# tphakala/birdnet-go

Measured on AMD Instinct MI355X. Metric: 3s-48kHz clips/sec (whole node) + max-abs prob diff vs TFLite, BirdNET v2.4, higher is better.
Workload: dtype f32; 1 GPU; BASELINE configs[1]: BirdNET v2.4 fp32, batch 256 x 3 s @ 48 kHz per GPU, mel front-end + CNN + head on device, raw logits out; batch_per_gpu=256, n_samples=144000, n_classes=6522, pipeline_depth=2, input_sets=4

## Files before the change

birdnet-go_amd/csrc/engine.cpp:

```cpp
#include "engine.h"

#include <algorithm>
#include <cmath>
#include <cstdio>
#include <cstdlib>
#include <cstring>
#include <mutex>
#include <sstream>

#include "../../include/bnhip.h"
#include "hostpipe.h"

namespace bnhip {

#define HIPCHK(call)                                                                           \
    do {                                                                                       \
        hipError_t e_ = (call);                                                                \
        if (e_ != hipSuccess) {                                                                \
            *err = std::string(#call) + ": " + hipGetErrorString(e_);                          \
            return false;                                                                      \
        }                                                                                      \
    } while (0)

Engine::~Engine() {
// ... 383 lines not shown
        if (s.kind == S_MEAN_FINISH && si > 1 && steps[si - 2].tail == 1 && tail_taken(si - 2, n, nl > 1)) continue;
        ProfEntry pe{};
        static const char* dbg_sync_before = getenv("BNHIP_DEBUG_SYNC_BEFORE");
        static const char* dbg_sync_after = getenv("BNHIP_DEBUG_SYNC_AFTER");
        static const char* dbg_ctx1_only = getenv("BNHIP_DEBUG_CTX1_ONLY");
        if (dbg_ctx1_only && cur_ctx == 1 && !strstr(dbg_ctx1_only, s.kclass)) continue;
        static const char* dbg_ctx1_skip = getenv("BNHIP_DEBUG_CTX1_SKIP");
        if (dbg_ctx1_skip && cur_ctx == 1 && strstr(dbg_ctx1_skip, s.kclass)) continue;
        if (dbg_sync_before && (!strcmp(dbg_sync_before, s.kclass) || s.name.rfind(dbg_sync_before, 0) == 0)) hipStreamSynchronize(stream);
        const bool prof_this = profiling && (profile_filter.empty() || profile_filter == s.kclass);
        if (prof_this) { pe.a = get_event(); pe.b = get_event(); pe.step = si; pe.n = n; hipEventRecord(pe.a, stream); }
        switch (s.kind) {
            case S_MINMAX:
                launch_clip_minmax(in0, n, n_samples, specs[0].eps, reinterpret_cast<float2*>(out),
                                   mm_scratch ? mm_scratch + ((size_t)std::max(cur_ctx, 0) * kMaxLanes + (size_t)li) * kMinMaxScratch : nullptr, stream);
                break;
            case S_FRONTEND: {
                const FrontSpec& fs = specs[s.spec];
                FrontendParams p;
                p.x = in0; p.mm = reinterpret_cast<const float2*>(in1); p.G = fs.G; p.window = fs.window; p.out = out;
                p.n_samples = n_samples; p.L = fs.L; p.Lfft = fs.Lfft; p.Kp = fs.Kp; p.hop = fs.hop; p.F = fs.F; p.n_mels = fs.n_mels;
                p.NTP = fs.NTP; p.C = C_spec; p.c = fs.c; p.norm_sub = fs.norm_sub; p.norm_mul = fs.norm_mul;
                p.p1 = fs.p1; p.p2 = fs.p2; p.n_clips = n;
                launch_frontend(p, stream);
                break;
            }
            case S_NORMALIZE:
                launch_normalize(in0, reinterpret_cast<const float2*>(in1), out, n, n_samples, specs[0].norm_sub, specs[0].norm_mul, stream);
                break;
            case S_STFT: {
                const FrontSpec& fs = specs[s.spec];
                StftParams p{in0, fs.window_full, fs.bins, out, n_samples, fs.Lfft, fs.L, fs.hop, fs.F, fs.nb, fs.nbp, fs.mode, n, fs.stft_tw, fs.pad_left};
                p.zmask = fs.stft_zmask;
                if (s.mode == 1) {
                    p.out = nullptr; p.img = out; p.mel = s.w3; p.mel_quads = s.S; p.n_mels = fs.n_mels; p.Ctot = C_spec; p.c0 = fs.c;
                    p.logc = fs.log_compress ? 1 : 0; p.time_major = fs.time_major ? 1 : 0; p.p1 = fs.p1; p.p2 = fs.p2;
                    p.lfloor = fs.log_floor; p.lscale = fs.log_scale;
                }
                {
                    static const bool f32_off = getenv("BNHIP_STFT_F32") && atoi(getenv("BNHIP_STFT_F32")) == 0;
                    if (precision == 1 && s.mode != 1 && fs.log_compress && !f32_off) p.f32 = 1;
                }
                launch_stft_bins(p, stream);
                break;
            }
            case S_MELBAND: {
                const FrontSpec& fa = specs[s.spec];
                const FrontSpec& fb = specs[s.S == 2 ? s.op : s.spec];
                MelBandParams p{{in0, s.S == 2 ? in1 : in0}, {s.w0, s.S == 2 ? s.w2 : s.w0},
                                {reinterpret_cast<const int*>(s.w1), reinterpret_cast<const int*>(s.S == 2 ? s.w3 : s.w1)},
                                {fa.nbp, fb.nbp}, {fa.p1, fb.p1}, {fa.p2, fb.p2}, out, fa.F, fa.n_mels, C_spec, fa.c,
                                fa.log_compress ? 1 : 0, fa.log_floor, fa.log_scale, fa.time_major ? 1 : 0};
                launch_mel_banded(p, s.S, n, stream);
                break;
            }
            case S_MELFIN: {
                const FrontSpec& fa = specs[s.spec];
                const FrontSpec& fb = specs[s.S == 2 ? s.op : s.spec];
                MelFinParams p{{in0, s.S == 2 ? in1 : in0}, {fa.p1, fb.p1}, {fa.p2, fb.p2}, out, fa.F, fa.n_mels, fa.n_mels, C_spec, fa.c,
                               fa.log_compress ? 1 : 0, fa.log_floor, fa.log_scale, fa.time_major ? 1 : 0};
                launch_mel_finish(p, s.S, n, stream);
                break;
            }
            case S_CONV_DIRECT: {
                ConvParams p{in0, s.w0, s.w1, out, n, s.H, s.W, s.C, s.Ho, s.Wo, s.Co, s.kh, s.kw, s.sh, s.sw, s.pt, s.pl, s.act};
                p.out_bf16 = vals[s.out].half ? 1 : 0;
// ... 137 lines not shown

static void jesc(std::ostringstream& os, const std::string& s) {
    for (char c : s) { if (c == '"' || c == '\\') os << '\\'; os << c; }
}

struct StepView { std::string name; double flops, bytes; bool absorbed; };
static StepView step_view(const Engine& e, size_t i) {
    const Step& s = e.steps[i];
    StepView v{s.name, s.flops, s.bytes, false};
    auto fused = [&](size_t k) { return e.steps[k].kind == S_PW && e.steps[k].tail && e.steps[k].wm_full >= 13; };
    if (fused(i)) {
        const double mine = 4.0 * s.H * s.W * s.Co;
        if (s.tail == 2) { v.name += "+dw"; v.flops += e.steps[i + 1].flops; }
        else { v.name += "+mean"; v.flops += e.steps[i + 1].flops + e.steps[i + 2].flops; v.bytes += 4.0 * s.Co - mine; }
    } else if ((s.kind == S_DW && i > 0 && e.steps[i - 1].tail == 2 && fused(i - 1)) ||
               (s.kind == S_MEAN_PARTIAL && i > 0 && e.steps[i - 1].tail == 1 && fused(i - 1)) ||
               (s.kind == S_MEAN_FINISH && i > 1 && e.steps[i - 2].tail == 1 && fused(i - 2))) {
        v.flops = 0; v.bytes = 0; v.absorbed = true;
    }
    return v;
}

std::string Engine::describe() const {
    std::ostringstream os;
    os << "{\"tune_source\":\"";
    jesc(os, tune_source);
    os << "\",\"tune_key\":\"" << (device >= 0 ? tune_key() : std::string()) << "\",\"split_step\":" << split_step << ",\"heatmap_tail\":\"" << (heatmap_pruned_step() >= 0 ? "pruned" : "gather") << "\",\"n_samples\":" << n_samples << ",\"n_classes\":" << n_classes << ",\"emb_dim\":" << emb_dim
       << ",\"max_batch\":" << max_batch << ",\"logits_output\":" << logits_output << ",\"embedding_output\":" << embedding_output << ",\"precision\":\"" << (precision ? "bf16" : "f32") << "\",\"lanes\":" << n_lanes << ",\"lane_min_batch\":" << dual_lane_min << ",\"act_arena_bytes\":" << act_bytes << ",\"weight_bytes\":" << w_bytes
       << ",\"specs\":[";
    for (size_t i = 0; i < specs.size(); i++) {
        const FrontSpec& f = specs[i];
        os << (i ? "," : "") << "{\"frame_length\":" << f.L << ",\"fft_length\":" << f.Lfft << ",\"hop\":" << f.hop
           << ",\"frames\":" << f.F << ",\"n_mels\":" << f.n_mels << ",\"channel\":" << f.c << ",\"p1\":" << f.p1
           << ",\"p2\":" << f.p2 << "}";
    }
    os << "],\"steps\":[";
    for (size_t i = 0; i < steps.size(); i++) {
        const Step& s = steps[i];
        const StepView sv = step_view(*this, i);
        const bool absorbed = sv.absorbed;
        os << (i ? "," : "") << "{\"i\":" << i << ",\"kernel\":\"" << s.kclass << "\",\"name\":\"";
        jesc(os, sv.name);
        os << "\",\"H\":" << s.H << ",\"W\":" << s.W << ",\"C\":" << s.C << ",\"Co\":" << s.Co << ",\"k\":" << s.kh
           << ",\"stride\":" << s.sh << ",\"act\":" << s.act << ",\"fused_scale\":" << (s.kind == S_PW && s.in1 >= 0 ? 1 : 0)
           << ",\"shape\":" << s.shape << ",\"dw_lds\":" << s.dwl << ",\"bx\":" << s.bx << ",\"nt\":" << s.nt << ",\"wm\":" << s.wm << ",\"nt_full\":" << s.nt_full << ",\"wm_full\":" << s.wm_full << ",\"fused_res\":" << (s.kind == S_PW && s.in2 >= 0 ? 1 : 0) << ",\"fused_sum\":" << (s.out2 >= 0 ? 1 : 0) << ",\"flops\":" << sv.flops << ",\"bytes\":" << sv.bytes << ",\"wbytes\":" << s.wbytes
           << ",\"tail\":" << s.tail << ",\"absorbed\":" << (absorbed ? 1 : 0) << ",\"out_v\":" << s.out << ",\"out2_v\":" << s.out2
           << ",\"in_bf16\":" << ((s.in0 >= 0 && vals[s.in0].half) ? 1 : 0) << ",\"out_bf16\":" << ((s.out >= 0 && vals[s.out].half) ? 1 : 0) << "}";
    }
    os << "]}";
    return os.str();
}

std::string Engine::profile_read() {
    hipStreamSynchronize(stream);
    struct Agg { double ms = 0, flops = 0, bytes = 0; long launches = 0; };
    std::map<std::string, Agg> agg;
    std::vector<std::string> order;
    std::vector<Agg> per_step(steps.size());
    for (auto& e : prof) {
        float ms = 0;
        hipEventElapsedTime(&ms, e.a, e.b);
        const Step& s = steps[e.step];
        const StepView sv = step_view(*this, e.step);
        if (!agg.count(s.kclass)) order.push_back(s.kclass);
        Agg& a = agg[s.kclass];
        a.ms += ms; a.launches++; a.flops += sv.flops * e.n; a.bytes += sv.bytes * e.n + s.wbytes;
        Agg& ps = per_step[e.step];
        ps.ms += ms; ps.launches++; ps.flops += sv.flops * e.n; ps.bytes += sv.bytes * e.n + s.wbytes;
        ev_pool.push_back(e.a); ev_pool.push_back(e.b);
    }
    prof.clear();
    std::ostringstream os;
    os << "[";
    for (size_t i = 0; i < order.size(); i++) {
        const Agg& a = agg[order[i]];
        os << (i ? "," : "") << "{\"kernel\":\"" << order[i] << "\",\"launches\":" << a.launches << ",\"ms\":" << a.ms
           << ",\"flops\":" << a.flops << ",\"bytes\":" << a.bytes << "}";
    }
    for (size_t i = 0; i < steps.size(); i++) {
        const Agg& a = per_step[i];
// ... 11 lines not shown
```

birdnet-go_amd/csrc/engine.h:

```cpp
#pragma once
#include <hip/hip_runtime.h>

#include <map>
#include <string>
#include <vector>

#include "kernels.h"
#include "tflite_model.h"

namespace bnhip {

enum StepKind { S_MINMAX, S_FRONTEND, S_NORMALIZE, S_STFT, S_MELFIN, S_MELBAND, S_CONV_DIRECT, S_PW, S_DW, S_EXPAND_DW, S_MEAN_PARTIAL, S_MEAN_FINISH, S_SE, S_UNARY, S_BINARY,
                S_EW_UNARY, S_EW_BINARY, S_POOL, S_COPY, S_SOFTMAX, S_REDUCE, S_CONV_GENERIC,
                S_CONV_IGEMM };

struct GenGeom {
    int d[4] = {1, 1, 1, 1};
    long sa[4] = {0, 0, 0, 0}, sb[4] = {0, 0, 0, 0}, so[4] = {0, 0, 0, 0};
    long offa = 0, offo = 0;
    bool a_const = false, b_const = false;
    int mask = 0;
    float alpha = 0.f;
    bool fill = false;
    int dh = 1, dw = 1, depthwise = 0, mult = 1;
// ... 10 lines not shown
    int bx = 0;
    int H = 0, W = 0, C = 0, Ho = 0, Wo = 0, Co = 0, kh = 1, kw = 1, sh = 1, sw = 1, pt = 0, pl = 0;
    int act = 0, act2 = 0, op = 0, mode = 0, S = 1, Cr = 0;
    int nt = 0, wm = 0;
    int tail = 0;
    int H2 = 0, W2 = 0, pt2 = 0, pl2 = 0;
    int shape = -1;
    int nt_full = 0, wm_full = 0;
    int spec = -1;
    GenGeom g;
    double flops = 0, bytes = 0, wbytes = 0;
};

struct Value {
    int tfl = -1;
    size_t elems = 0;
    size_t offset = 0;
    size_t offset_lane = 0;
    int first = -1, last = -1;
    bool external = false;
    bool half = false;
};

struct FrontSpec {
    int L, Kp, Lfft, hop, F, n_mels, NTP, c;
    float p1, p2, eps, norm_sub, norm_mul;
    const double* G = nullptr;
    const float* window = nullptr;
    bool fft = false;
    int nb = 0, nbp = 0, mode = 0;
    const float* window_full = nullptr;
    const double* stft_tw = nullptr;
    unsigned stft_zmask = 0xffffffffu;
    const int* bins = nullptr;
    bool normalize = true, log_compress = false, time_major = false;
    int pad_left = 0;
    float log_floor = 0.f, log_scale = 1.f;
};

struct ProfEntry { hipEvent_t a, b; int step; int n; };

struct WeightPlan {
    std::vector<float> img;
    std::vector<size_t> step_w[4];
    std::vector<size_t> step_bx;
};

inline DwParams dw_params(const Step& s, const float* in = nullptr, float* out = nullptr, int n = 1) {
    return DwParams{in, s.w0, s.w1, out, n, s.H, s.W, s.C, s.Ho, s.Wo, s.kh, s.kw, s.sh, s.sw, s.pt, s.pl, s.act};
}
PwTail tail_of(const Step& s, const Step& c);

class Engine {
  public:
    ~Engine();
    bool build(TflModel m, int device, int max_batch, bool plan_only, std::string* err, int* code);
    bool run(const float* d_in, int n, float* d_logits, float* d_emb, std::string* err);

    int device = 0, max_batch = 256;
    bool no_reuse = false;
    bool autotune = true;
    bool defer_weights = false;
    void finish_deferred();
    char* weights_ptr() const { return w_arena; }
    size_t weights_bytes() const { return w_bytes; }
    int frontend_fft = -1;
// ... 114 lines not shown
```

birdnet-go_amd/csrc/kernels.h:

```cpp
#pragma once
#include <atomic>
#include <hip/hip_runtime.h>

#include <vector>
#include <cstdint>

namespace bnhip {

inline int device_cus() {
    static std::atomic<int> cus[64];
    int dev = 0;
    if (hipGetDevice(&dev) != hipSuccess) { (void)hipGetLastError(); return 256; }
    if (dev < 0 || dev >= 64) return 256;
    int c = cus[dev].load(std::memory_order_relaxed);
    if (c > 0) return c;
    hipDeviceProp_t pr{};
    if (hipGetDeviceProperties(&pr, dev) != hipSuccess || pr.multiProcessorCount <= 0) { (void)hipGetLastError(); return 256; }
    cus[dev].store(pr.multiProcessorCount, std::memory_order_relaxed);
    return pr.multiProcessorCount;
}

template <auto Kern>
inline void lds_limit_once(int bytes) {
    static std::atomic<unsigned long long> done{0};
// ... 9 lines not shown

enum Act : int { ACT_NONE = 0, ACT_RELU = 1, ACT_RELU_N1_TO_1 = 2, ACT_RELU6 = 3, ACT_TANH = 4, ACT_SWISH = 100, ACT_SIGMOID = 101, ACT_HARD_SWISH = 102 };

void launch_pcm_to_f32(const void* pcm, int bits , float* out, size_t n, hipStream_t s);

constexpr int kMinMaxParts = 16;
void launch_clip_minmax(const float* x, int n_clips, int n_samples, float eps, float2* mm, float* scratch , hipStream_t s);

struct FrontendParams {
    const float* x;
    const float2* mm;
    const double* G;
    const float* window;
    float* out;
    int n_samples, L, Lfft, Kp, hop, F, n_mels, NTP, C, c;
    float norm_sub, norm_mul;
    float p1, p2;
    int n_clips;
};
void launch_frontend(const FrontendParams& p, hipStream_t s);
size_t frontend_lds_bytes(int Lfft, int Kp, int hop, int NTP);

struct StftParams {
    const float* xn;
    const float* window;
    const int* bins;
    float* out;
    int n_samples, Lfft, L, hop, F, nb, nbp, mode , n_clips;
    const double* tw = nullptr;
    int pad_left = 0;
    int nb_cap = 0, fpw = 0;
    int f32 = 0;
    unsigned zmask = 0xffffffffu;
    const float* mel = nullptr;
    int mel_quads = 0, n_mels = 0, Ctot = 1, c0 = 0, logc = 0, time_major = 0;
    float p1 = 1.f, p2 = 1.f, lfloor = 0.f, lscale = 1.f;
    float* img = nullptr;
};
std::vector<double> stft_build_tables(int Lfft, const int* bins, int nb);
unsigned stft_zmask(int Lfft, const int* bins, int nb);
std::vector<float> stft_mel_table(int Lfft, const float* melw, const int* span, int n_mels, int nb, int nbp, int* quads);
void launch_normalize(const float* x, const float2* mm, float* out, int n_clips, int n_samples, float norm_sub,
                      float norm_mul, hipStream_t s);
bool stft_supported(int Lfft, int nb);
void launch_stft_bins(const StftParams& p, hipStream_t s);
struct MelFinParams {
    const float* T[2];
    float p1[2], p2[2];
    float* out;
    int F, n_mels, ldt, Ctot, c0;
    int log = 0;
    float lfloor = 0.f, lscale = 1.f;
    int time_major = 0;
};
void launch_mel_finish(const MelFinParams& p, int nch, int n_clips, hipStream_t s);
struct MelBandParams {
    const float* bins[2];
    const float* w[2];
    const int* span[2];
    int nbp[2];
    float p1[2], p2[2];
    float* out;
    int F, n_mels, Ctot, c0;
    int log = 0;
    float lfloor = 0.f, lscale = 1.f;
    int time_major = 0;
};
bool mel_banded_supported(int n_mels, int nbp0, int nbp1);
void launch_mel_banded(const MelBandParams& p, int nch, int n_clips, hipStream_t s);
int frontend_kc(int Lfft, int hop, int NTP);

struct ConvParams {
    const float* in; const float* w ; const float* bias; float* out;
// ... 152 lines not shown
```

birdnet-go_amd/csrc/planner.cpp:

```cpp
#include "engine.h"

#include <algorithm>
#include <cmath>
#include <cstdio>
#include <cstdlib>
#include <cstring>
#include <map>

#include "../../include/bnhip.h"

namespace bnhip {

namespace {

size_t align_up(size_t v, size_t a) { return (v + a - 1) / a * a; }

struct Planner {
    const TflModel& m;
    std::vector<int> producer;
    std::vector<std::vector<int>> consumers;
    std::vector<int> uses;
    std::vector<char> absorbed;
    std::string err;

// ... 260 lines not shown
        return P.fail("front-end: unexpected spectrogram tensor shape");
    fm->out_tensor = t;
    return true;
}

std::vector<double> build_G(const Planner& P, const FrontendMatch& fm, const std::vector<int>& krows, int Kp, int NTP) {
    const int nb = fm.Lfft / 2 + 1, nm = fm.n_mels, N = fm.Lfft;
    const float* melT = P.T(fm.mel_tensor).f32();
    std::vector<double> ctab(N);
    for (int i = 0; i < N; i++) ctab[i] = std::cos(2.0 * M_PI * (double)i / (double)N);
    std::vector<double> melk(krows.size() * (size_t)nm);
    for (size_t r = 0; r < krows.size(); r++)
        for (int mm = 0; mm < nm; mm++) melk[r * nm + mm] = (double)melT[(size_t)mm * nb + krows[r]];
    std::vector<double> G((size_t)Kp * NTP, 0.0);
    std::vector<double> row(nm);
    for (int n = 0; n <= fm.Lfft / 2; n++) {
        std::fill(row.begin(), row.end(), 0.0);
        for (size_t r = 0; r < krows.size(); r++) {
            double c = ctab[(size_t)(((long long)krows[r] * n) % N)];
            const double* mk = &melk[r * nm];
            for (int mm = 0; mm < nm; mm++) row[mm] += c * mk[mm];
        }
        for (int mo = 0; mo < nm; mo++) {
            int mm = fm.reverse ? nm - 1 - mo : mo;
            G[(size_t)n * NTP + mo] = row[mm];
        }
    }
    return G;
}

struct PlanSwitches {
    bool mel_banded = !getenv("BNHIP_NO_MEL_BANDED");
    bool fuse_mel = getenv("BNHIP_FUSE_MEL") != nullptr;
    bool fuse_expdw = !(getenv("BNHIP_NO_FUSE_EXPDW") && atoi(getenv("BNHIP_NO_FUSE_EXPDW")) != 0);
    bool conv_igemm = !getenv("BNHIP_NO_CONV_IGEMM");
    bool stem_mfma = !getenv("BNHIP_NO_STEM_MFMA");
    bool fuse_stem = !getenv("BNHIP_NO_FUSE_STEM");
};

int map_act(int fused, int* post = nullptr) {
    if (post) *post = 0;
    switch (fused) {
        case 0: return ACT_NONE; case 1: return ACT_RELU; case 3: return ACT_RELU6;
        case 2: if (post) { *post = U_RELU_N1_TO_1; return ACT_NONE; } return -1;
        case 4: if (post) { *post = U_TANH; return ACT_NONE; } return -1;
        default: return -1;
    }
}

void conv_pads(const TflOp& o, int H, int W, int Ho, int Wo, int kh, int kw, int* pt, int* pl) {
    *pt = 0; *pl = 0;
    if (o.explicit_pad) { *pt = o.pad_t; *pl = o.pad_l; return; }
    if (o.padding == 0) {
        *pt = std::max((Ho - 1) * o.stride_h + (kh - 1) * o.dil_h + 1 - H, 0) / 2;
        *pl = std::max((Wo - 1) * o.stride_w + (kw - 1) * o.dil_w + 1 - W, 0) / 2;
    }
}

bool shape5(const std::vector<int>& sh, int out[5]) {
    std::vector<int> v = sh;
    while (v.size() > 5 && v[0] == 1) v.erase(v.begin());
    if (v.size() > 5) return false;
    for (int k = 0; k < 5; k++) out[k] = 1;
    for (size_t k = 0; k < v.size(); k++) out[5 - v.size() + k] = v[k];
    return out[0] == 1;
}
// ... 237 lines not shown
            add_step(nz);
        }
        fs.nb = (int)bins.size(); fs.nbp = (int)align_up(fs.nb, 4); fs.mode = fm.magnitude ? 1 : 0;
        const int nbins = fm.Lfft / 2 + 1;
        const float* melT = P.T(fm.mel_tensor).f32();
        std::vector<float> melw((size_t)fm.n_mels * fs.nbp, 0.f);
        for (int mo = 0; mo < fm.n_mels; mo++) {
            int mm = fm.reverse ? fm.n_mels - 1 - mo : mo;
            for (int r = 0; r < fs.nb; r++) melw[(size_t)mo * fs.nbp + r] = melT[(size_t)mm * nbins + bins[r]];
        }
        const size_t o_win = wpush(fm.window), o_bins = wpush_i32(bins);
        const size_t o_mel = wpush(melw);
        std::vector<double> twt = stft_build_tables(fm.Lfft, bins.data(), fs.nb);
        fs.stft_zmask = stft_zmask(fm.Lfft, bins.data(), fs.nb);
        const size_t o_tw = wpush(reinterpret_cast<const float*>(twt.data()), twt.size() * 2);
        specs.push_back(fs);
        const int si = (int)specs.size() - 1;
        std::vector<int> span((size_t)2 * fm.n_mels, 0);
        long span_sum = 0;
        for (int mo = 0; mo < fm.n_mels; mo++) {
            int lo = fs.nb, hi = 0;
            for (int r = 0; r < fs.nb; r++)
                if (melw[(size_t)mo * fs.nbp + r] != 0.0f) { lo = std::min(lo, r); hi = r + 1; }
            if (hi == 0) lo = 0;
            span[2 * mo] = lo; span[2 * mo + 1] = hi;
            span_sum += hi - lo;
        }
        const size_t o_span = wpush_i32(span);
        const bool banded = sw.mel_banded && span_sum * 4 <= (long)fm.n_mels * fs.nb;
        int mel_quads = 0;
        std::vector<float> meltab;
        if (banded && sw.fuse_mel) meltab = stft_mel_table(fm.Lfft, melw.data(), span.data(), fm.n_mels, fs.nb, fs.nbp, &mel_quads);
        const bool fused = !meltab.empty();
        int v_bins = fused ? -1 : new_val(-1, (size_t)fm.F * fs.nbp);
        Step st; st.kind = S_STFT; st.name = "stft" + std::to_string(i); st.kclass = "stft"; st.in0 = v_xn; st.out = fused ? v_spec : v_bins;
        st.spec = si;
        st.flops = (double)fm.F * 2.5 * fm.Lfft * std::log2((double)fm.Lfft / 2);
        st.bytes = (double)E.n_samples * 4 + (double)fm.F * (fused ? fm.n_mels : fs.nbp) * 4;
        if (fused) { st.mode = 1; st.S = mel_quads; st.name += "+mel"; st.flops += 4.0 * fm.F * fs.nb; }
        add_step(st, o_win, o_bins, o_tw, fused ? wpush(meltab) : SIZE_MAX);
        fft_fin.push_back({v_bins, si, o_mel, o_span, banded, fused});
        return true;
    }
    bool gemm_channel(int i, FrontSpec fs, const std::vector<int>& bins) {
        const FrontendMatch& fm = fms[i];
        std::vector<double> G = build_G(P, fm, bins, fs.Kp, fs.NTP);
        const size_t goff = wpush(reinterpret_cast<const float*>(G.data()), G.size() * 2);
        std::vector<float> wpad((size_t)2 * fs.Kp, 0.0f);
        for (int n = 0; n <= fm.Lfft / 2; n++) {
            if (n < fm.L) wpad[n] = fm.window[n];
            int mi = fm.Lfft - n;
            if (n > 0 && mi != n && mi < fm.L) wpad[fs.Kp + n] = fm.window[mi];
        }
        const size_t woff = wpush(wpad);
        specs.push_back(fs);
        Step f; f.kind = S_FRONTEND; f.name = "melspec" + std::to_string(i); f.kclass = "frontend";
        f.in0 = E.v_input; f.in1 = E.v_mm; f.out = v_spec; f.spec = (int)specs.size() - 1;
        f.flops = 2.0 * fm.F * (fm.Lfft / 2 + 1) * fm.n_mels;
        f.bytes = (double)E.n_samples * 4 + (double)fm.F * fm.n_mels * 4;
        return add_step(f, goff, woff);
    }
    void mel_finish() {
        for (size_t k = 0; k < fft_fin.size();) {
            if (fft_fin[k].fused) { k++; continue; }
            const FrontSpec& a = specs[fft_fin[k].spec];
            const FrontSpec* b = k + 1 < fft_fin.size() && !fft_fin[k + 1].fused ? &specs[fft_fin[k + 1].spec] : nullptr;
// ... 856 lines not shown
```

birdnet-go_amd/csrc/stft.hip:

```cpp
#include "kernels.h"

#include <hip/hip_runtime.h>

#include <algorithm>
#include <vector>
#include <cmath>
#include <cstdio>
#include <cstdlib>

namespace bnhip {

__global__ void k_normalize(const float* __restrict__ x, const float2* __restrict__ mm, float* __restrict__ out,
                            int n_samples, float norm_sub, float norm_mul) {
    const int b = blockIdx.y;
    const float2 m = mm[b];
    const float* xc = x + (size_t)b * n_samples;
    float* oc = out + (size_t)b * n_samples;
    for (int i = blockIdx.x * blockDim.x + threadIdx.x; i < n_samples; i += gridDim.x * blockDim.x) {
        float t = xc[i] - m.x;
        t = t / m.y;
        t = t - norm_sub;
        oc[i] = t * norm_mul;
    }
}
// ... 12 lines not shown
    constexpr int LOG = P == 16 ? 4 : (P == 8 ? 3 : (P == 4 ? 2 : 1));
#pragma unroll
    for (int i = 0; i < P; i++) {
        int j = 0;
#pragma unroll
        for (int bit = 0; bit < LOG; bit++) j |= ((i >> bit) & 1) << (LOG - 1 - bit);
        if (i < j) { R t = re[i]; re[i] = re[j]; re[j] = t; t = im[i]; im[i] = im[j]; im[j] = t; }
    }
#pragma unroll
    for (int len = 2; len <= P; len <<= 1) {
        const int half = len >> 1, step = 16 / len;
#pragma unroll
        for (int i = 0; i < P; i += len) {
#pragma unroll
            for (int k = 0; k < half; k++) {
                const R wr = (R)C16[k * step], wi = (R)-S16[k * step];
                const R xr = re[i + k + half], xi = im[i + k + half];
                const R ur = re[i + k], ui = im[i + k];
                if (k == 0) {
                    re[i + k] = ur + xr; im[i + k] = ui + xi; re[i + k + half] = ur - xr; im[i + k + half] = ui - xi;
                } else if (2 * k == half) {
                    re[i + k] = ur + xi; im[i + k] = ui - xr; re[i + k + half] = ur - xi; im[i + k + half] = ui + xr;
                } else {
                    re[i + k] = fma(xr, wr, fma(-xi, wi, ur));
                    im[i + k] = fma(xr, wi, fma(xi, wr, ui));
                    re[i + k + half] = fma(-xr, wr, fma(xi, wi, ur));
                    im[i + k + half] = fma(-xr, wi, fma(-xi, wr, ui));
                }
            }
        }
    }
}

__device__ __forceinline__ float mel_pow(float v, float p1, float p2);
__device__ __forceinline__ float mel_log(float v, float lfloor, float lscale);

template <int P, int W, bool MEL = false, typename R = double>
__global__ __launch_bounds__(64 * W) void k_stft_bins(StftParams p) {
    constexpr int N2 = 64 * P;
    constexpr int N = 2 * N2;
    constexpr int Q = 64 / P;
    constexpr int RS = P == 8 ? 66 : 65;
    constexpr int WSZ = P * RS;
    constexpr int NPAIR = (P * P + 63) / 64;
    extern __shared__ __attribute__((aligned(16))) unsigned char stft_sm[];
    R* sm = reinterpret_cast<R*>(stft_sm);
    R* twr = sm;
    R* twi = twr + P * 64;
    R* t2r = twi + P * 64;
    R* t2i = t2r + Q * P;
    R* work = t2i + Q * P;
    float4* melw4 = reinterpret_cast<float4*>(work + (size_t)W * 2 * WSZ);
    const int* binq = reinterpret_cast<const int*>(melw4 + p.mel_quads);
    const int tid = threadIdx.x, lane = tid & 63, wave = tid >> 6;
    const int b = blockIdx.y;

    constexpr int NTAB = 2 * P * 64 + 2 * Q * P;
    for (int i = tid; i < NTAB; i += blockDim.x) sm[i] = (R)p.tw[i];
    int mA = 0, loA = 0, nA = 0, wA = 0, mB = 0, loB = 0, nB = 0, wB = 0;
    if (MEL) {
        const float4* src = reinterpret_cast<const float4*>(p.mel + 64 * 8);
        for (int i = tid; i < p.mel_quads + (p.mel_quads + 3) / 4; i += blockDim.x) melw4[i] = src[i];
        const int4* lt = reinterpret_cast<const int4*>(p.mel) + 2 * lane;
        const int4 ta = lt[0], tb = lt[1];
        mA = ta.x; loA = ta.y; nA = ta.z; wA = ta.w; mB = tb.x; loB = tb.y; nB = tb.z; wB = tb.w;
    }
    __syncthreads();

    R* wre = work + (size_t)wave * 2 * WSZ;
    R* wim = wre + WSZ;
    const float* xc = p.xn + (size_t)b * p.n_samples;
    float w0[P], w1[P];
#pragma unroll
    for (int n1 = 0; n1 < P; n1++) {
        int n = 128 * n1 + 2 * lane;
        w0[n1] = n < p.L ? p.window[n] : 0.f;
        w1[n1] = n + 1 < p.L ? p.window[n + 1] : 0.f;
    }
    const int k1b = lane % P, qb = lane / P;
    constexpr int NBL = 8;
    int ka_[NBL], kb_[NBL];
    R trr[NBL], tri[NBL];
#pragma unroll
    for (int t = 0; t < NBL; t++) {
        int idx = lane + 64 * t;
        int k = idx < p.nb ? p.bins[idx] : 0;
        ka_[t] = k % N2; kb_[t] = (N2 - k % N2) % N2;
        const bool in = idx < p.nb_cap;
        trr[t] = in ? (R)p.tw[NTAB + idx] : (R)1.0;
        tri[t] = in ? (R)p.tw[NTAB + p.nb_cap + idx] : (R)0.0;
    }

    const int f_begin = (blockIdx.x * W + wave) * p.fpw;
    const int f_end = min(f_begin + p.fpw, p.F);
    float2 nx[P];
    auto fetch = [&](int f) {
        const int first = f * p.hop - p.pad_left;
        const int s0 = first + 2 * lane;
        if (first >= 0 && first + N <= p.n_samples && (first & 1) == 0) {
#pragma unroll
            for (int n1 = 0; n1 < P; n1++)
                nx[n1] = 128 * n1 < p.L ? *reinterpret_cast<const float2*>(xc + s0 + 128 * n1) : make_float2(0.f, 0.f);
        } else {
#pragma unroll
            for (int n1 = 0; n1 < P; n1++) {
                int s = s0 + 128 * n1;
                float2 v = make_float2(0.f, 0.f);
                if (128 * n1 < p.L) {
                    if (s >= 0 && s < p.n_samples) v.x = xc[s];
                    if (s + 1 >= 0 && s + 1 < p.n_samples) v.y = xc[s + 1];
                }
                nx[n1] = v;
            }
        }
    };
    if (f_begin < f_end) fetch(f_begin);
    for (int f = f_begin; f < f_end; f++) {
        R re[P], im[P];
#pragma unroll
        for (int n1 = 0; n1 < P; n1++) {
            re[n1] = (R)(nx[n1].x * w0[n1]);
            im[n1] = (R)(nx[n1].y * w1[n1]);
        }
        if (f + 1 < f_end) fetch(f + 1);
        fft_regs<P, R>(re, im);
#pragma unroll
        for (int k1 = 0; k1 < P; k1++) {
            const R c = twr[k1 * 64 + lane], s = twi[k1 * 64 + lane];
            const R r = fma(re[k1], c, -(im[k1] * s)), i2 = fma(re[k1], s, im[k1] * c);
            wre[k1 * RS + lane] = r; wim[k1 * RS + lane] = i2;
        }
        __builtin_amdgcn_s_waitcnt(0xc07f);
        __builtin_amdgcn_wave_barrier();
#pragma unroll
        for (int j = 0; j < P; j++) { re[j] = wre[k1b * RS + Q * j + qb]; im[j] = wim[k1b * RS + Q * j + qb]; }
        __builtin_amdgcn_s_waitcnt(0xc07f);
        __builtin_amdgcn_wave_barrier();
        fft_regs<P, R>(re, im);
#pragma unroll
        for (int j = 0; j < P; j++) {
            const R c = t2r[qb * P + j], s = t2i[qb * P + j];
            const R r = fma(re[j], c, -(im[j] * s)), i2 = fma(re[j], s, im[j] * c);
            const int slot = j * P + k1b;
            wre[qb * (P * P) + slot] = r; wim[qb * (P * P) + slot] = i2;
        }
        __builtin_amdgcn_s_waitcnt(0xc07f);
        __builtin_amdgcn_wave_barrier();
        R ar[NPAIR][Q], ai[NPAIR][Q];
#pragma unroll
        for (int t = 0; t < NPAIR; t++) {
            const int slot = min(lane + 64 * t, P * P - 1);
#pragma unroll
            for (int q = 0; q < Q; q++) { ar[t][q] = wre[q * (P * P) + slot]; ai[t][q] = wim[q * (P * P) + slot]; }
        }
        __builtin_amdgcn_s_waitcnt(0xc07f);
        __builtin_amdgcn_wave_barrier();
#pragma unroll
        for (int t = 0; t < NPAIR; t++) {
            const int slot = lane + 64 * t;
            const int kbase = (slot % P) + P * (slot / P);
            const unsigned zm = Q == 4 ? (p.zmask >> (4 * t)) & 15u : 15u;
            if (Q == 4 && zm != 15u) {
                if (slot < P * P) {
                    if (zm & 5u) {
                        const R a_r = ar[t][0] + ar[t][2], a_i = ai[t][0] + ai[t][2], c_r = ar[t][1] + ar[t][3], c_i = ai[t][1] + ai[t][3];
                        if (zm & 1u) { wre[kbase] = a_r + c_r; wim[kbase] = a_i + c_i; }
                        if (zm & 4u) { wre[kbase + 2 * P * P] = a_r - c_r; wim[kbase + 2 * P * P] = a_i - c_i; }
                    }
                    if (zm & 10u) {
                        const R b_r = ar[t][0] - ar[t][2], b_i = ai[t][0] - ai[t][2], d_r = ar[t][1] - ar[t][3], d_i = ai[t][1] - ai[t][3];
                        if (zm & 2u) { wre[kbase + P * P] = b_r + d_i; wim[kbase + P * P] = b_i - d_r; }
                        if (zm & 8u) { wre[kbase + 3 * P * P] = b_r - d_i; wim[kbase + 3 * P * P] = b_i + d_r; }
                    }
                }
                continue;
            }
            fft_regs<Q, R>(ar[t], ai[t]);
            if (slot < P * P) {
#pragma unroll
                for (int q = 0; q < Q; q++) { wre[kbase + P * P * q] = ar[t][q]; wim[kbase + P * P * q] = ai[t][q]; }
            }
        }
        __builtin_amdgcn_s_waitcnt(0xc07f);
        __builtin_amdgcn_wave_barrier();
        float* orow = MEL ? nullptr : p.out + ((size_t)b * p.F + f) * p.nbp;
        float ov[NBL];
#pragma unroll
        for (int t = 0; t < NBL; t++) {
            const int idx = lane + 64 * t;
            ov[t] = 0.f;
            if (idx >= p.nbp) break;
            float o = 0.f;
            if (idx < p.nb) {
                const int ka = ka_[t], kb = kb_[t];
                const R zr = wre[ka], zi = wim[ka], mr = wre[kb], mi = -wim[kb];
                const R er = (R)0.5 * (zr + mr), ei = (R)0.5 * (zi + mi);
                const R dr = zr - mr, di = zi - mi;
                const R or_ = (R)0.5 * di, oi = (R)-0.5 * dr;
                const R c = trr[t], s = tri[t];
                const R xr = er + fma(or_, c, -(oi * s));
                if (p.mode == 0) o = (float)xr;
                else {
                    const R xi = ei + fma(or_, s, oi * c);
                    o = hypotf((float)xr, (float)xi);
                }
            }
            if (MEL) ov[t] = o; else orow[idx] = o;
        }
        if (MEL) {
            __builtin_amdgcn_s_waitcnt(0xc07f);
            __builtin_amdgcn_wave_barrier();
            float* brow = reinterpret_cast<float*>(wre);
#pragma unroll
            for (int t = 0; t < NBL; t++) { const int idx = lane + 64 * t; if (idx < p.nbp) brow[idx] = ov[t]; }
            __builtin_amdgcn_s_waitcnt(0xc07f);
            __builtin_amdgcn_wave_barrier();
            const float4* b4 = reinterpret_cast<const float4*>(brow);
            float* part = brow + 512;
            for (int e = lane; e < p.mel_quads; e += 64) {
                const float4 x4 = b4[binq[e]], w4 = melw4[e];
                part[e] = fmaf(x4.w, w4.w, fmaf(x4.z, w4.z, fmaf(x4.y, w4.y, x4.x * w4.x)));
            }
            __builtin_amdgcn_s_waitcnt(0xc07f);
            __builtin_amdgcn_wave_barrier();
            (void)loA; (void)loB;
#pragma unroll 1
            for (int which = 0; which < 2; which++) {
                const int mm = which ? mB : mA, n4 = which ? nB : nA, wo = which ? wB : wA;
                if (n4 < 0) continue;
                float acc = 0.f;
                for (int g = 0; g < n4; g += 4) {
                    const float t0 = part[wo + g], t1 = g + 1 < n4 ? part[wo + g + 1] : 0.f, t2 = g + 2 < n4 ? part[wo + g + 2] : 0.f,
                                t3 = g + 3 < n4 ? part[wo + g + 3] : 0.f;
                    acc = (((acc + t0) + t1) + t2) + t3;
                }
                const float v = p.logc ? mel_log(acc, p.lfloor, p.lscale) : mel_pow(acc, p.p1, p.p2);
                const size_t o = p.time_major ? (((size_t)b * p.F + f) * p.n_mels + mm) * p.Ctot + p.c0
                                              : (((size_t)b * p.n_mels + mm) * p.F + f) * p.Ctot + p.c0;
                p.img[o] = v;
            }
        }
        for (int idx = lane + 64 * NBL; !MEL && idx < p.nbp; idx += 64) {
            float o = 0.f;
            if (idx < p.nb) {
                const int k = p.bins[idx];
                const int ka = k % N2, kb = (N2 - k % N2) % N2;
                const R zr = wre[ka], zi = wim[ka], mr = wre[kb], mi = -wim[kb];
                const R er = (R)0.5 * (zr + mr), ei = (R)0.5 * (zi + mi);
                const R dr = zr - mr, di = zi - mi;
                const R or_ = (R)0.5 * di, oi = (R)-0.5 * dr;
                const R c = (R)p.tw[NTAB + idx], s = (R)p.tw[NTAB + p.nb_cap + idx];
                const R xr = er + fma(or_, c, -(oi * s));
                if (p.mode == 0) o = (float)xr;
                else {
                    const R xi = ei + fma(or_, s, oi * c);
                    o = hypotf((float)xr, (float)xi);
                }
            }
            orow[idx] = o;
        }
        __builtin_amdgcn_s_waitcnt(0xc07f);
        __builtin_amdgcn_wave_barrier();
    }
}

std::vector<double> stft_build_tables(int Lfft, const int* bins, int nb) {
    const int P = Lfft / 128, Q = 64 / P, N2 = 64 * P, cap = (nb + 63) / 64 * 64;
    const double tau = -6.283185307179586476925286766559;
    std::vector<double> t((size_t)2 * P * 64 + 2 * Q * P + 2 * cap);
    double* twr = t.data();
    double* twi = twr + P * 64;
    double* t2r = twi + P * 64;
    double* t2i = t2r + Q * P;
    double* trr = t2i + Q * P;
    double* tri = trr + cap;
    for (int i = 0; i < P * 64; i++) {
        const double a = tau * (double)(((i >> 6) * (i & 63)) % N2) / (double)N2;
        twr[i] = std::cos(a); twi[i] = std::sin(a);
    }
    for (int i = 0; i < Q * P; i++) {
        const double a = tau * (double)(((i / P) * (i % P)) % 64) / 64.0;
        t2r[i] = std::cos(a); t2i[i] = std::sin(a);
    }
    for (int i = 0; i < cap; i++) {
        const double a = tau * (double)(i < nb ? bins[i] : 0) / (double)Lfft;
        trr[i] = std::cos(a); tri[i] = std::sin(a);
    }
    return t;
}
unsigned stft_zmask(int Lfft, const int* bins, int nb) {
    const char* e = getenv("BNHIP_STFT_PRUNE");
    const bool off = e && atoi(e) == 0;
    const int P = Lfft / 128;
    if (P != 16 || off || nb <= 0) return 0xffffffffu;
    const int N2 = 64 * P;
    unsigned m = 0;
    auto need = [&](int z) { const int qp = z / (P * P), slot = ((z % (P * P)) / P) * P + z % P; m |= 1u << (4 * (slot / 64) + qp); };
    for (int i = 0; i < nb; i++) { const int k = bins[i] % N2; need(k); need((N2 - k) % N2); }
    return m | 0xffff0000u;
}
static int stft_waves(int P) { return P == 8 ? 4 : 8; }
size_t stft_lds_bytes(int P, int nb_cap) {
    (void)nb_cap;
    return (size_t)(2 * P * 64 + 2 * (64 / P) * P + stft_waves(P) * 2 * P * (P == 8 ? 66 : 65)) * sizeof(double);
}
bool stft_supported(int Lfft, int nb) {
    if (Lfft != 2048 && Lfft != 1024 && Lfft != 512) return false;
    int P = Lfft / 128, cap = (nb + 63) / 64 * 64;
    return nb <= Lfft / 2 + 1 && stft_lds_bytes(P, cap) <= 160 * 1024;
}
std::vector<float> stft_mel_table(int Lfft, const float* melw, const int* span, int n_mels, int nb, int nbp, int* quads) {
    *quads = 0;
    if (n_mels < 1 || n_mels > 128 || nbp > 512 || nb > nbp || (nbp & 3)) return {};
    std::vector<int> lo4(n_mels), n4(n_mels), wo(n_mels);
    int tot = 0;
    for (int m = 0; m < n_mels; m++) {
        const int lo = span[2 * m], hi = span[2 * m + 1];
        lo4[m] = lo >> 2; n4[m] = hi > lo ? ((hi + 3) >> 2) - (lo >> 2) : 0; wo[m] = tot;
        tot += n4[m];
    }
    const int P = Lfft / 128;
    if (stft_lds_bytes(P, 0) + (size_t)tot * 16 + (size_t)(tot + 3) / 4 * 16 > 160 * 1024) return {};
    if (nbp > 512 || tot > 256) return {};
    std::vector<float> t((size_t)64 * 8 + (size_t)tot * 4 + (size_t)(tot + 3) / 4 * 4, 0.f);
    int* lt = reinterpret_cast<int*>(t.data());
    const int half = (n_mels + 1) / 2;
    for (int l = 0; l < 64; l++) {
        int* e = lt + 8 * l;
        e[2] = e[6] = -1;
        if (l >= half) continue;
        const int a = l, bnd = n_mels - 1 - l;
        e[0] = a; e[1] = lo4[a]; e[2] = n4[a]; e[3] = wo[a];
        if (bnd != a) { e[4] = bnd; e[5] = lo4[bnd]; e[6] = n4[bnd]; e[7] = wo[bnd]; }
    }
    for (int m = 0; m < n_mels; m++)
        for (int g = 0; g < n4[m]; g++)
            for (int q = 0; q < 4; q++) {
                const int k = 4 * (lo4[m] + g) + q;
                t[(size_t)64 * 8 + 4 * ((size_t)wo[m] + g) + q] = k < nbp ? melw[(size_t)m * nbp + k] : 0.f;
            }
    int* bq = reinterpret_cast<int*>(t.data() + (size_t)64 * 8 + (size_t)tot * 4);
    for (int m = 0; m < n_mels; m++)
        for (int g = 0; g < n4[m]; g++) bq[wo[m] + g] = lo4[m] + g;
    *quads = tot;
    return t;
}
void launch_stft_bins(const StftParams& p0, hipStream_t s) {
    StftParams p = p0;
    p.nb_cap = (p.nb + 63) / 64 * 64;
    static int fpw_env = getenv("BNHIP_STFT_FPW") ? atoi(getenv("BNHIP_STFT_FPW")) : 0;
    long waves_wanted = 2048;
    long fpw = fpw_env > 0 ? fpw_env : ((long)p.F * p.n_clips + waves_wanted - 1) / waves_wanted;
    p.fpw = (int)std::min<long>(std::max<long>(fpw, 1), 16);
    const int P = p.Lfft / 128, W = stft_waves(P);
    size_t lds = stft_lds_bytes(P, p.nb_cap);
    dim3 grid((p.F + W * p.fpw - 1) / (W * p.fpw), p.n_clips);
    if (p.mel) {
        lds += (size_t)p.mel_quads * 16 + (size_t)(p.mel_quads + 3) / 4 * 16;
        if (P == 16) {
            lds_limit_once<&k_stft_bins<16, 8, true>>(160 * 1024);
            hipLaunchKernelGGL((k_stft_bins<16, 8, true>), grid, dim3(64 * W), lds, s, p);
        } else if (P == 8) {
            lds_limit_once<&k_stft_bins<8, 4, true>>(160 * 1024);
            hipLaunchKernelGGL((k_stft_bins<8, 4, true>), grid, dim3(64 * W), lds, s, p);
        } else {
            lds_limit_once<&k_stft_bins<4, 8, true>>(160 * 1024);
            hipLaunchKernelGGL((k_stft_bins<4, 8, true>), grid, dim3(64 * W), lds, s, p);
        }
        return;
    }
    if (p.f32) {
        lds /= 2;
        if (P == 4) hipLaunchKernelGGL((k_stft_bins<4, 8, false, float>), grid, dim3(64 * W), lds, s, p);
        else if (P == 16) {
            lds_limit_once<&k_stft_bins<16, 8, false, float>>(160 * 1024);
            hipLaunchKernelGGL((k_stft_bins<16, 8, false, float>), grid, dim3(64 * W), lds, s, p);
        } else hipLaunchKernelGGL((k_stft_bins<8, 4, false, float>), grid, dim3(64 * W), lds, s, p);
        return;
    }
    if (P == 4) {
        hipLaunchKernelGGL((k_stft_bins<4, 8>), grid, dim3(64 * W), lds, s, p);
    } else if (P == 16) {
        lds_limit_once<&k_stft_bins<16, 8>>(160 * 1024);
        hipLaunchKernelGGL((k_stft_bins<16, 8>), grid, dim3(64 * W), lds, s, p);
    } else {
        hipLaunchKernelGGL((k_stft_bins<8, 4>), grid, dim3(64 * W), lds, s, p);
    }
}

__device__ __forceinline__ float mel_pow(float v, float p1, float p2) {
    float y = (p1 == 2.0f) ? v * v : powf(v, p1);
    if (p2 == 1.0f) return y;
    if (y >= 0.0f) return y == 0.0f ? 0.0f : __builtin_amdgcn_exp2f(p2 * __builtin_amdgcn_logf(y));
    return powf(y, p2);
}
__device__ __forceinline__ float mel_log(float v, float lfloor, float lscale) {
    return lscale * (0.6931471805599453f * __builtin_amdgcn_logf(fmaxf(v, lfloor)));
}
template <int C>
__global__ __launch_bounds__(256) void k_mel_finish(MelFinParams p) {
    __shared__ float tile[C][32][33];
    const int b = blockIdx.z, f0 = blockIdx.x * 32, m0 = blockIdx.y * 32;
    const int tx = threadIdx.x & 31, ty = threadIdx.x >> 5;
#pragma unroll
    for (int c = 0; c < C; c++)
        for (int r = ty; r < 32; r += 8) {
            int f = f0 + r, m = m0 + tx;
            float v = 0.f;
            if (f < p.F && m < p.n_mels) {
                const float t = p.T[c][((size_t)b * p.F + f) * p.ldt + m];
                v = p.log ? mel_log(t, p.lfloor, p.lscale) : mel_pow(t, p.p1[c], p.p2[c]);
            }
// ... 135 lines not shown
```

Baseline: 77280 clips/s.

## Compute two STFT frames per complex FFT via paired real-signal trick

Result: slower. 73910 clips/s (-4.4%).

```diff
diff --git a/birdnet-go_amd/csrc/engine.cpp b/birdnet-go_amd/csrc/engine.cpp
--- a/birdnet-go_amd/csrc/engine.cpp
+++ b/birdnet-go_amd/csrc/engine.cpp
@@ -439,6 +439,7 @@
                 const FrontSpec& fs = specs[s.spec];
                 StftParams p{in0, fs.window_full, fs.bins, out, n_samples, fs.Lfft, fs.L, fs.hop, fs.F, fs.nb, fs.nbp, fs.mode, n, fs.stft_tw, fs.pad_left};
                 p.zmask = fs.stft_zmask;
+                p.pair = fs.stft_pair ? 1 : 0; p.pair_special = fs.stft_pair_special ? 1 : 0;
                 if (s.mode == 1) {
                     p.out = nullptr; p.img = out; p.mel = s.w3; p.mel_quads = s.S; p.n_mels = fs.n_mels; p.Ctot = C_spec; p.c0 = fs.c;
                     p.logc = fs.log_compress ? 1 : 0; p.time_major = fs.time_major ? 1 : 0; p.p1 = fs.p1; p.p2 = fs.p2;
@@ -642,7 +643,8 @@
         const FrontSpec& f = specs[i];
         os << (i ? "," : "") << "{\"frame_length\":" << f.L << ",\"fft_length\":" << f.Lfft << ",\"hop\":" << f.hop
            << ",\"frames\":" << f.F << ",\"n_mels\":" << f.n_mels << ",\"channel\":" << f.c << ",\"p1\":" << f.p1
-           << ",\"p2\":" << f.p2 << "}";
+           << ",\"p2\":" << f.p2 << ",\"needed_bins\":" << f.nb << ",\"stft_pair\":" << (f.stft_pair ? 1 : 0)
+           << ",\"stft_pair_special\":" << (f.stft_pair && f.stft_pair_special ? 1 : 0) << "}";
     }
     os << "],\"steps\":[";
     for (size_t i = 0; i < steps.size(); i++) {
@@ -655,7 +657,9 @@
            << ",\"stride\":" << s.sh << ",\"act\":" << s.act << ",\"fused_scale\":" << (s.kind == S_PW && s.in1 >= 0 ? 1 : 0)
            << ",\"shape\":" << s.shape << ",\"dw_lds\":" << s.dwl << ",\"bx\":" << s.bx << ",\"nt\":" << s.nt << ",\"wm\":" << s.wm << ",\"nt_full\":" << s.nt_full << ",\"wm_full\":" << s.wm_full << ",\"fused_res\":" << (s.kind == S_PW && s.in2 >= 0 ? 1 : 0) << ",\"fused_sum\":" << (s.out2 >= 0 ? 1 : 0) << ",\"flops\":" << sv.flops << ",\"bytes\":" << sv.bytes << ",\"wbytes\":" << s.wbytes
            << ",\"tail\":" << s.tail << ",\"absorbed\":" << (absorbed ? 1 : 0) << ",\"out_v\":" << s.out << ",\"out2_v\":" << s.out2
-           << ",\"in_bf16\":" << ((s.in0 >= 0 && vals[s.in0].half) ? 1 : 0) << ",\"out_bf16\":" << ((s.out >= 0 && vals[s.out].half) ? 1 : 0) << "}";
+           << ",\"in_bf16\":" << ((s.in0 >= 0 && vals[s.in0].half) ? 1 : 0) << ",\"out_bf16\":" << ((s.out >= 0 && vals[s.out].half) ? 1 : 0);
+        if (s.kind == S_STFT) os << ",\"stft_form\":\"" << (specs[s.spec].stft_pair && s.mode != 1 ? "paired" : "per-frame") << "\"";
+        os << "}";
     }
     os << "]}";
     return os.str();
diff --git a/birdnet-go_amd/csrc/engine.h b/birdnet-go_amd/csrc/engine.h
--- a/birdnet-go_amd/csrc/engine.h
+++ b/birdnet-go_amd/csrc/engine.h
@@ -66,6 +66,7 @@
     const float* window_full = nullptr;
     const double* stft_tw = nullptr;
     unsigned stft_zmask = 0xffffffffu;
+    bool stft_pair = false, stft_pair_special = false;
     const int* bins = nullptr;
     bool normalize = true, log_compress = false, time_major = false;
     int pad_left = 0;
diff --git a/birdnet-go_amd/csrc/kernels.h b/birdnet-go_amd/csrc/kernels.h
--- a/birdnet-go_amd/csrc/kernels.h
+++ b/birdnet-go_amd/csrc/kernels.h
@@ -65,6 +65,7 @@
     int nb_cap = 0, fpw = 0;
     int f32 = 0;
     unsigned zmask = 0xffffffffu;
+    int pair = 0, pair_special = 0;
     const float* mel = nullptr;
     int mel_quads = 0, n_mels = 0, Ctot = 1, c0 = 0, logc = 0, time_major = 0;
     float p1 = 1.f, p2 = 1.f, lfloor = 0.f, lscale = 1.f;
@@ -72,6 +73,8 @@
 };
 std::vector<double> stft_build_tables(int Lfft, const int* bins, int nb);
 unsigned stft_zmask(int Lfft, const int* bins, int nb);
+bool stft_pair_special(int Lfft, const int* bins, int nb);
+bool stft_pair_enabled();
 std::vector<float> stft_mel_table(int Lfft, const float* melw, const int* span, int n_mels, int nb, int nbp, int* quads);
 void launch_normalize(const float* x, const float2* mm, float* out, int n_clips, int n_samples, float norm_sub,
                       float norm_mul, hipStream_t s);
diff --git a/birdnet-go_amd/csrc/planner.cpp b/birdnet-go_amd/csrc/planner.cpp
--- a/birdnet-go_amd/csrc/planner.cpp
+++ b/birdnet-go_amd/csrc/planner.cpp
@@ -316,6 +316,7 @@
 struct PlanSwitches {
     bool mel_banded = !getenv("BNHIP_NO_MEL_BANDED");
     bool fuse_mel = getenv("BNHIP_FUSE_MEL") != nullptr;
+    bool stft_pair = stft_pair_enabled();
     bool fuse_expdw = !(getenv("BNHIP_NO_FUSE_EXPDW") && atoi(getenv("BNHIP_NO_FUSE_EXPDW")) != 0);
     bool conv_igemm = !getenv("BNHIP_NO_CONV_IGEMM");
     bool stem_mfma = !getenv("BNHIP_NO_STEM_MFMA");
@@ -619,6 +620,8 @@
         std::vector<float> meltab;
         if (banded && sw.fuse_mel) meltab = stft_mel_table(fm.Lfft, melw.data(), span.data(), fm.n_mels, fs.nb, fs.nbp, &mel_quads);
         const bool fused = !meltab.empty();
+        specs[si].stft_pair = sw.stft_pair && !fused && fs.mode == 0 && E.precision == 0;
+        specs[si].stft_pair_special = stft_pair_special(fm.Lfft, bins.data(), fs.nb);
         int v_bins = fused ? -1 : new_val(-1, (size_t)fm.F * fs.nbp);
         Step st; st.kind = S_STFT; st.name = "stft" + std::to_string(i); st.kclass = "stft"; st.in0 = v_xn; st.out = fused ? v_spec : v_bins;
         st.spec = si;
diff --git a/birdnet-go_amd/csrc/stft.hip b/birdnet-go_amd/csrc/stft.hip
--- a/birdnet-go_amd/csrc/stft.hip
+++ b/birdnet-go_amd/csrc/stft.hip
@@ -68,11 +68,17 @@
     }
 }
 
+template <int CTRL>
+__device__ __forceinline__ float lane_move(float old, float v) {
+    return __int_as_float(__builtin_amdgcn_update_dpp(__float_as_int(old), __float_as_int(v), CTRL, 0xf, 0xf, false));
+}
+
 __device__ __forceinline__ float mel_pow(float v, float p1, float p2);
 __device__ __forceinline__ float mel_log(float v, float lfloor, float lscale);
 
-template <int P, int W, bool MEL = false, typename R = double>
-__global__ __launch_bounds__(64 * W) void k_stft_bins(StftParams p) {
+template <int P, int W, bool MEL = false, typename R = double, bool PAIR = false, int NBL = 8>
+__global__ __launch_bounds__(64 * W, (PAIR && P == 8) ? 3 : 1) void k_stft_bins(StftParams p) {
+    static_assert(!PAIR || (!MEL && sizeof(R) == 8), "the paired form is fp64, bins to HBM");
     constexpr int N2 = 64 * P;
     constexpr int N = 2 * N2;
     constexpr int Q = 64 / P;
@@ -114,7 +120,6 @@
         w1[n1] = n + 1 < p.L ? p.window[n + 1] : 0.f;
     }
     const int k1b = lane % P, qb = lane / P;
-    constexpr int NBL = 8;
     int ka_[NBL], kb_[NBL];
     R trr[NBL], tri[NBL];
 #pragma unroll
@@ -129,11 +134,14 @@
 
     const int f_begin = (blockIdx.x * W + wave) * p.fpw;
     const int f_end = min(f_begin + p.fpw, p.F);
-    float2 nx[P];
-    auto fetch = [&](int f) {
+    float2 nx[P], ny[PAIR ? P : 1];
+    auto fetch = [&](int f, float2* nx) {
         const int first = f * p.hop - p.pad_left;
         const int s0 = first + 2 * lane;
-        if (first >= 0 && first + N <= p.n_samples && (first & 1) == 0) {
+        if (PAIR && f >= p.F) {
+#pragma unroll
+            for (int n1 = 0; n1 < P; n1++) nx[n1] = make_float2(0.f, 0.f);
+        } else if (first >= 0 && first + N <= p.n_samples && (first & 1) == 0) {
 #pragma unroll
             for (int n1 = 0; n1 < P; n1++)
                 nx[n1] = 128 * n1 < p.L ? *reinterpret_cast<const float2*>(xc + s0 + 128 * n1) : make_float2(0.f, 0.f);
@@ -150,15 +158,64 @@
             }
         }
     };
-    if (f_begin < f_end) fetch(f_begin);
-    for (int f = f_begin; f < f_end; f++) {
+    if (f_begin < f_end) { fetch(f_begin, nx); if (PAIR) fetch(f_begin + 1, ny); }
+    for (int f = f_begin; f < f_end; f += PAIR ? 2 : 1) {
         R re[P], im[P];
+        R sb0 = (R)0.0, sb1 = (R)0.0;
+        if constexpr (!PAIR) {
 #pragma unroll
         for (int n1 = 0; n1 < P; n1++) {
             re[n1] = (R)(nx[n1].x * w0[n1]);
             im[n1] = (R)(nx[n1].y * w1[n1]);
         }
-        if (f + 1 < f_end) fetch(f + 1);
+        if (f + 1 < f_end) fetch(f + 1, nx);
+        } else {
+        float a0[P], a1[P], b0[P], b1[P];
+#pragma unroll
+        for (int n1 = 0; n1 < P; n1++) {
+            a0[n1] = nx[n1].x * w0[n1]; a1[n1] = nx[n1].y * w1[n1];
+            b0[n1] = ny[n1].x * w0[n1]; b1[n1] = ny[n1].y * w1[n1];
+        }
+        if (p.pair_special) {
+#pragma unroll
+            for (int n1 = 0; n1 < P; n1++) { sb0 += (R)b0[n1] + (R)b1[n1]; sb1 += (R)b0[n1] - (R)b1[n1]; }
+#pragma unroll
+            for (int m = 1; m < 64; m <<= 1) { sb0 += __shfl_xor(sb0, m); sb1 += __shfl_xor(sb1, m); }
+        }
+        auto halves = [&](int n, R& p0, R& p1, R& m0, R& m1) {
+            const float bm = lane_move<0x138>(lane_move<0x13C>(0.f, b1[(n + P - 1) % P]), b1[n]);
+            const float bp = lane_move<0x130>(lane_move<0x134>(0.f, b0[(n + 1) % P]), b0[n]);
+            const R v0 = (R)b1[n] - (R)bm, v1 = (R)bp - (R)b0[n];
+            const R u0 = (R)a0[n], u1 = (R)a1[n];
+            p0 = u0 + v0; p1 = u1 + v1; m0 = u0 - v0; m1 = u1 - v1;
+        };
+        const int rev = (63 - lane) * 4;
+        auto mirror = [&](R v) {
+            return __hiloint2double(__builtin_amdgcn_ds_bpermute(rev, __double2hiint(v)), __builtin_amdgcn_ds_bpermute(rev, __double2loint(v)));
+        };
+        auto mirror_up = [&](R v) {
+            const R r = mirror(v);
+            return __hiloint2double(__builtin_amdgcn_update_dpp(0, __double2hiint(r), 0x138, 0xf, 0xf, true),
+                                    __builtin_amdgcn_update_dpp(0, __double2loint(r), 0x138, 0xf, 0xf, true));
+        };
+        R own[P];
+#pragma unroll
+        for (int n1 = 0; n1 < P / 2; n1++) {
+            const int c = P - 1 - n1;
+            R pa0, pa1, ma0, ma1, pc0, pc1, mc0, mc1;
+            halves(n1, pa0, pa1, ma0, ma1);
+            halves(c, pc0, pc1, mc0, mc1);
+            own[n1] = __hiloint2double(__builtin_amdgcn_readfirstlane(__double2hiint(ma0)), __builtin_amdgcn_readfirstlane(__double2loint(ma0)));
+            own[c] = __hiloint2double(__builtin_amdgcn_readfirstlane(__double2hiint(mc0)), __builtin_amdgcn_readfirstlane(__double2loint(mc0)));
+            re[n1] = pa0 + mirror_up(mc0); im[n1] = pa1 + mirror(mc1);
+            re[c] = pc0 + mirror_up(ma0); im[c] = pc1 + mirror(ma1);
+        }
+        if (lane == 0) {
+#pragma unroll
+            for (int n1 = 0; n1 < P; n1++) re[n1] += own[(P - n1) % P];
+        }
+        if (f + 2 < f_end) { fetch(f + 2, nx); fetch(f + 3, ny); }
+        }
         fft_regs<P, R>(re, im);
 #pragma unroll
         for (int k1 = 0; k1 < P; k1++) {
@@ -220,13 +277,14 @@
         __builtin_amdgcn_s_waitcnt(0xc07f);
         __builtin_amdgcn_wave_barrier();
         float* orow = MEL ? nullptr : p.out + ((size_t)b * p.F + f) * p.nbp;
+        const bool has_b = PAIR && f + 1 < p.F;
         float ov[NBL];
 #pragma unroll
         for (int t = 0; t < NBL; t++) {
             const int idx = lane + 64 * t;
             ov[t] = 0.f;
             if (idx >= p.nbp) break;
-            float o = 0.f;
+            float o = 0.f, o2 = 0.f;
             if (idx < p.nb) {
                 const int ka = ka_[t], kb = kb_[t];
                 const R zr = wre[ka], zi = wim[ka], mr = wre[kb], mi = -wim[kb];
@@ -235,13 +293,19 @@
                 const R or_ = (R)0.5 * di, oi = (R)-0.5 * dr;
                 const R c = trr[t], s = tri[t];
                 const R xr = er + fma(or_, c, -(oi * s));
-                if (p.mode == 0) o = (float)xr;
+                if (PAIR) {
+                    const R xi = ei + fma(or_, s, oi * c);
+                    o = (float)((R)0.5 * xr);
+                    o2 = (float)(((R)0.5 * xi) * (R)p.tw[NTAB + 2 * p.nb_cap + idx]);
+                    if (p.pair_special && ka == 0) o2 = (float)(c > (R)0.0 ? sb0 : sb1);
+                } else if (p.mode == 0) o = (float)xr;
                 else {
                     const R xi = ei + fma(or_, s, oi * c);
                     o = hypotf((float)xr, (float)xi);
                 }
             }
             if (MEL) ov[t] = o; else orow[idx] = o;
+            if (has_b) orow[p.nbp + idx] = o2;
         }
         if (MEL) {
             __builtin_amdgcn_s_waitcnt(0xc07f);
@@ -277,7 +341,7 @@
             }
         }
         for (int idx = lane + 64 * NBL; !MEL && idx < p.nbp; idx += 64) {
-            float o = 0.f;
+            float o = 0.f, o2 = 0.f;
             if (idx < p.nb) {
                 const int k = p.bins[idx];
                 const int ka = k % N2, kb = (N2 - k % N2) % N2;
@@ -287,13 +351,19 @@
                 const R or_ = (R)0.5 * di, oi = (R)-0.5 * dr;
                 const R c = (R)p.tw[NTAB + idx], s = (R)p.tw[NTAB + p.nb_cap + idx];
                 const R xr = er + fma(or_, c, -(oi * s));
-                if (p.mode == 0) o = (float)xr;
+                if (PAIR) {
+                    const R xi = ei + fma(or_, s, oi * c);
+                    o = (float)((R)0.5 * xr);
+                    o2 = (float)(((R)0.5 * xi) * (R)p.tw[NTAB + 2 * p.nb_cap + idx]);
+                    if (p.pair_special && ka == 0) o2 = (float)(c > (R)0.0 ? sb0 : sb1);
+                } else if (p.mode == 0) o = (float)xr;
                 else {
                     const R xi = ei + fma(or_, s, oi * c);
                     o = hypotf((float)xr, (float)xi);
                 }
             }
             orow[idx] = o;
+            if (has_b) orow[p.nbp + idx] = o2;
         }
         __builtin_amdgcn_s_waitcnt(0xc07f);
         __builtin_amdgcn_wave_barrier();
@@ -303,13 +373,14 @@
 std::vector<double> stft_build_tables(int Lfft, const int* bins, int nb) {
     const int P = Lfft / 128, Q = 64 / P, N2 = 64 * P, cap = (nb + 63) / 64 * 64;
     const double tau = -6.283185307179586476925286766559;
-    std::vector<double> t((size_t)2 * P * 64 + 2 * Q * P + 2 * cap);
+    std::vector<double> t((size_t)2 * P * 64 + 2 * Q * P + 3 * cap);
     double* twr = t.data();
     double* twi = twr + P * 64;
     double* t2r = twi + P * 64;
     double* t2i = t2r + Q * P;
     double* trr = t2i + Q * P;
     double* tri = trr + cap;
+    double* i2s = tri + cap;
     for (int i = 0; i < P * 64; i++) {
         const double a = tau * (double)(((i >> 6) * (i & 63)) % N2) / (double)N2;
         twr[i] = std::cos(a); twi[i] = std::sin(a);
@@ -321,8 +392,19 @@
     for (int i = 0; i < cap; i++) {
         const double a = tau * (double)(i < nb ? bins[i] : 0) / (double)Lfft;
         trr[i] = std::cos(a); tri[i] = std::sin(a);
+        const int k = i < nb ? bins[i] : 0;
+        i2s[i] = k > 0 && 2 * k < Lfft ? 1.0 / (2.0 * std::sin(-tau * (double)k / (double)Lfft)) : 0.0;
     }
     return t;
+}
+bool stft_pair_special(int Lfft, const int* bins, int nb) {
+    for (int i = 0; i < nb; i++)
+        if (bins[i] == 0 || 2 * bins[i] == Lfft) return true;
+    return false;
+}
+bool stft_pair_enabled() {
+    const char* e = getenv("BNHIP_STFT_PAIR");
+    return !(e && atoi(e) == 0);
 }
 unsigned stft_zmask(int Lfft, const int* bins, int nb) {
     const char* e = getenv("BNHIP_STFT_PRUNE");
@@ -388,6 +470,8 @@
     long waves_wanted = 2048;
     long fpw = fpw_env > 0 ? fpw_env : ((long)p.F * p.n_clips + waves_wanted - 1) / waves_wanted;
     p.fpw = (int)std::min<long>(std::max<long>(fpw, 1), 16);
+    const bool pair = p.pair && !p.mel && !p.f32 && p.mode == 0;
+    if (pair) p.fpw = (p.fpw + 1) & ~1;
     const int P = p.Lfft / 128, W = stft_waves(P);
     size_t lds = stft_lds_bytes(P, p.nb_cap);
     dim3 grid((p.F + W * p.fpw - 1) / (W * p.fpw), p.n_clips);
@@ -414,6 +498,18 @@
         } else hipLaunchKernelGGL((k_stft_bins<8, 4, false, float>), grid, dim3(64 * W), lds, s, p);
         return;
     }
+    if (pair) {
+        const int nbl = p.nb_cap <= 192 ? 3 : (p.nb_cap <= 320 ? 5 : 8);
+#define STFT_PAIR_LAUNCH(P_, W_, NBL_) \
+        do { lds_limit_once<&k_stft_bins<P_, W_, false, double, true, NBL_>>(160 * 1024); \
+             hipLaunchKernelGGL((k_stft_bins<P_, W_, false, double, true, NBL_>), grid, dim3(64 * W), lds, s, p); } while (0)
+#define STFT_PAIR_NBL(P_, W_) \
+        do { if (nbl == 3) STFT_PAIR_LAUNCH(P_, W_, 3); else if (nbl == 5) STFT_PAIR_LAUNCH(P_, W_, 5); else STFT_PAIR_LAUNCH(P_, W_, 8); } while (0)
+        if (P == 4) STFT_PAIR_NBL(4, 8); else if (P == 16) STFT_PAIR_NBL(16, 8); else STFT_PAIR_NBL(8, 4);
+#undef STFT_PAIR_NBL
+#undef STFT_PAIR_LAUNCH
+        return;
+    }
     if (P == 4) {
         hipLaunchKernelGGL((k_stft_bins<4, 8>), grid, dim3(64 * W), lds, s, p);
     } else if (P == 16) {
```
